# yangjames/Calico

Measured on AMD Instinct MI355X. Metric: LM iterations/sec on the 4-cam+IMU ~100k-observation problem, higher is better.
Workload: dtype f64

## Files before the change

calico_amd/csrc/bcr_kernels.hip:

```cpp
#include <hip/hip_runtime.h>

#include <algorithm>
#include <cassert>
#include <mutex>
#include <type_traits>

#include "kernels.hpp"
#include "problem_dev.hpp"
#include "solve_dev.hpp"
#include "block_elim.hpp"

namespace cal {

namespace {
constexpr int BP = kBcrBP;
constexpr int BB = BP * BP;
constexpr int DLD = 33;
constexpr int XLD = 2 * BP + kBcrFS + 1;
constexpr int CA = 0, CB = BP, CF = 2 * BP;
constexpr int kLevelThreads = 512;
constexpr int kLevelCodePrefetchBytes = 40 * 1024;
}

template <bool NEG, int NK>
// ... 63 lines not shown
struct Handoff { int* word; int seq; };
DEVI double load_sc1(const double* p) { return __hip_atomic_load(p, __ATOMIC_RELAXED, __HIP_MEMORY_SCOPE_AGENT); }
DEVI void store_sc1(double* p, double v) { __hip_atomic_store(p, v, __ATOMIC_RELAXED, __HIP_MEMORY_SCOPE_AGENT); }
template <bool HO> DEVI double load_y(const double* p) { return HO ? load_sc1(p) : *p; }
DEVI void handoff_publish(const Handoff& h) {
  asm volatile("s_waitcnt vmcnt(0)" ::: "memory");
  __syncthreads();
  if (threadIdx.x == 0) __hip_atomic_store(h.word, h.seq, __ATOMIC_RELAXED, __HIP_MEMORY_SCOPE_AGENT);
}
DEVI void fanin_arrive(int* word) {
  asm volatile("s_waitcnt vmcnt(0)" ::: "memory");
  __syncthreads();
  if (threadIdx.x == 0) __hip_atomic_fetch_add(word, 1, __ATOMIC_RELAXED, __HIP_MEMORY_SCOPE_AGENT);
}
DEVI void fanin_wait(const int* word, int n) {
  if (threadIdx.x == 0) {
    while (__hip_atomic_load(word, __ATOMIC_RELAXED, __HIP_MEMORY_SCOPE_AGENT) < n) __builtin_amdgcn_s_sleep(4);
  }
  __syncthreads();
}
DEVI void handoff_wait(const Handoff& h) {
  if (threadIdx.x == 0) {
    while (__hip_atomic_load(h.word, __ATOMIC_RELAXED, __HIP_MEMORY_SCOPE_AGENT) != h.seq) __builtin_amdgcn_s_sleep(4);
  }
  __syncthreads();
}

template <int NW, bool LATE>
DEVI void schur_tile(const SolveArgs& a, const BcrArgs& b, const FromR& fr, int tile, int slice, int ks, double* sacc ,
                     const int* fan_word, int n_prod, int late0, int late1) {
  const int mc = a.mc, m = a.m, m1 = a.m + 1, m1p = b.m1p, m1y = a.mc + 1;
  const int tid = threadIdx.x, lane = tid & 63, wave = tid >> 6;
  const size_t msq = size_t(m1) * m1;
  const int n = b.N * BP;
  int tr = 0, rem = tile;
  while (rem > tr) { rem -= tr + 1; ++tr; }
  const int tc = rem;
  const int lc16 = lane & 15, lk = lane >> 4;
  const int rows_per = ((n + ks - 1) / ks + 15) & ~15;
  const int r_begin = slice * rows_per, r_end = min(n, r_begin + rows_per);
  const int per_wave = (((r_end - r_begin + NW - 1) / NW + 3) / 4) * 4;
  const int w_begin = r_begin + wave * per_wave, w_end = min(r_end, w_begin + per_wave);
  const int ca = 16 * tr + lc16, cb = 16 * tc + lc16;
  const double* pa = b.Y + ca;
  const double* pb = b.Y + cb;
  const int f0 = LATE ? late0 : -1, f1 = LATE ? late1 : -1;
  double s0_pre = 0.0;
  if (tid < 256) {
    const int r = tr * 16 + (tid >> 4), c = tc * 16 + (tid & 15);
    if (r < m1y && c <= r && slice == 0) {
      if (r < mc) {
        s0_pre = a.R[a.off_C() + size_t(r) * mc + c];
        if (r == c) { const double d = fr.damping(s0_pre, a.n_s() + r); a.dadd[a.n_s() + r] = d; s0_pre += d; }
      } else if (c < mc) s0_pre = a.R[a.off_g() + a.n_s() + c];
    }
  }
  f64x4 acc = {0.0, 0.0, 0.0, 0.0};
  for (int kg = w_begin; kg < w_end; kg += 128) {
    double va[4][8], vb[4][8];
#pragma unroll
    for (int g = 0; g < 4; ++g) {
#pragma unroll
      for (int u = 0; u < 8; ++u) {
        const int row = kg + 32 * g + 4 * u + lk;
        const size_t ro = size_t(min(row, n - 1)) * m1p;
        va[g][u] = pa[ro]; vb[g][u] = pb[ro];
      }
    }
#pragma unroll
    for (int g = 0; g < 4; ++g) {
#pragma unroll
      for (int u = 0; u < 8; ++u) {
        const int row = kg + 32 * g + 4 * u + lk, sb = row >> 5;
        const bool use = row < w_end && sb != f0 && sb != f1;
        acc = __builtin_amdgcn_mfma_f64_16x16x4f64(use ? va[g][u] : 0.0, use ? vb[g][u] : 0.0, acc, 0, 0, 0);
      }
    }
  }
  if (LATE) {
    fanin_wait(fan_word, n_prod);
#pragma unroll
    for (int f = 0; f < 2; ++f) {
      const int sb = f == 0 ? f0 : f1;
      const int row = BP * max(sb, 0) + 4 * wave + lk;
      const bool use = sb >= 0 && wave < 8 && row >= r_begin && row < r_end;
      const size_t ro = size_t(min(row, n - 1)) * m1p;
      const double va = load_sc1(pa + ro), vb = load_sc1(pb + ro);
      acc = __builtin_amdgcn_mfma_f64_16x16x4f64(use ? va : 0.0, use ? vb : 0.0, acc, 0, 0, 0);
    }
  }
#pragma unroll
  for (int r = 0; r < 4; ++r) sacc[wave * 256 + (lk + 4 * r) * 16 + lc16] = acc[r];
  __syncthreads();
  if (tid < 256) {
    const int ti = tid >> 4, tj = tid & 15;
    const int r = tr * 16 + ti, c = tc * 16 + tj;
    double sum = 0.0;
#pragma unroll
    for (int w = 0; w < NW; ++w) sum += sacc[w * 256 + tid];
    if (r < m1y && c <= r) {
      const int fi = r < mc ? r : m, fc = c < mc ? c : m;
      a.Spart[size_t(slice) * msq + size_t(fi) * m1 + fc] = s0_pre - sum;
    }
  }
}
template <bool SC1>
DEVI void schur_root_rows(const SolveArgs& a, const BcrArgs& b, int ks, int w0, int nw, int NT) {
  if (b.root < 0) return;
  const int mc = a.mc, m = a.m, m1 = a.m + 1, m1p = b.m1p, m1y = a.mc + 1;
  const size_t msq = size_t(m1) * m1;
  const int tid = threadIdx.x;
  const int br = m - mc;
  const size_t fblk = size_t(BP) * m1p;
  const double* pD = b.pendD + size_t(b.root_par) * size_t(b.N) * 2 * BB;
  const double* pF = b.pendF + size_t(b.root_par) * size_t(b.N) * 2 * fblk;
  const int mask = b.root_pend;
  const int total = br * (m1y + br);
  auto ld = [](const double* p) { return SC1 ? load_sc1(p) : *p; };
  for (int e = w0 * NT + tid; e < total; e += nw * NT) {
    const int r = e / (m1y + br), j = e % (m1y + br);
    const bool in_f = j < m1y;
    const int r2 = j - m1y;
    if (!in_f && r2 > r) continue;
    const size_t o = in_f ? size_t(r) * m1p + j : size_t(r) * BP + r2;
    const double* base = in_f ? b.F + size_t(b.root) * fblk : b.D + size_t(b.root) * BB;
    const double* p0 = in_f ? pF + (size_t(b.root) * 2 + 0) * fblk : pD + (size_t(b.root) * 2 + 0) * BB;
    const double* p1 = in_f ? pF + (size_t(b.root) * 2 + 1) * fblk : pD + (size_t(b.root) * 2 + 1) * BB;
    const double v0 = ld(base + o), v1 = ld(p0 + o), v2 = ld(p1 + o);
    const double v = (v0 + ((mask & 1) ? v1 : 0.0)) + ((mask & 2) ? v2 : 0.0);
    int fi, fc;
    if (in_f) { if (j < mc) { fi = mc + r; fc = j; } else { fi = m; fc = mc + r; } }
    else { fi = mc + r; fc = mc + r2; }
    a.Spart[size_t(fi) * m1 + fc] = v;
    for (int k = 1; k < ks; ++k) a.Spart[size_t(k) * msq + size_t(fi) * m1 + fc] = 0.0;
  }
}

constexpr int kBcrTri = BP * (BP + 1) / 2;
template <int NL_, int NU_, int NF_>
struct BcrLoadMap {
  static constexpr int NL = NL_, NU = NU_, NF = NF_;
  static constexpr int NUD = (kBcrTri + NL_ - 1) / NL_;
  static_assert(NUD <= NU_ && NU_ <= 8 && NF_ <= 8, "BcrLoadMap: per-thread entry counts must fit the arrays and the flag bytes");
  int lt;
  int iD[NU_], iB[NU_];
  int rcD[NU_];
  bool okD[NU_], okB[NU_];
};
template <int NU, int NF>
struct BcrPre { double d[NU], bt[NU], at[NU], f[NF]; };
template <int NUD, int NU, int NF>
struct BcrRaw { double vraw[NUD], svv[NUD], q2v[NUD], vraw1[NUD], graw[NU], garaw[NU], graw1[NU], garaw1[NU], fraw[NF], fraw1[NF]; unsigned flags; };
constexpr int kRollTabWords = 48;
__device__ unsigned g_roll_tab[6][64][kRollTabWords];
static void fill_roll_table(unsigned (*tab)[64][kRollTabWords]) {
  constexpr int RB = 6 * kBcrCps;
  for (int k = 1; k <= 6; ++k) {
    auto pos = [&](int hi, int lo, bool& ok) {
      const int d = hi / 6 - lo / 6;
      ok = d < k;
      return unsigned(8 * (((lo / 6) * k + (ok ? d : 0)) * 36 + (lo % 6) * 6 + hi % 6));
    };
    for (int lane = 0; lane < 64; ++lane) {
      unsigned* t = tab[k - 1][lane];
      for (int i = 0; i < kRollTabWords; ++i) t[i] = 0;
      const int l16 = lane & 15, lk = lane >> 4;
      unsigned okS = 0, okB = 0, okA = 0;
      for (int r = 0; r < 4; ++r) {
        const int c = lk + 4 * r, hi = std::max(l16, c), lo = std::min(l16, c);
        bool ok;
        t[r] = pos(hi, lo, ok); if (ok) okS |= 1u << r;
        t[4 + r] = pos(16 + l16, c, ok); if (ok && 16 + l16 < RB) okS |= 1u << (4 + r);
        t[8 + r] = pos(16 + hi, 16 + lo, ok); if (ok && 16 + hi < RB) okS |= 1u << (8 + r);
      }
      for (int qt = 0; qt < 2; ++qt)
        for (int h = 0; h < 2; ++h)
          for (int r = 0; r < 4; ++r) {
            const int e = (qt * 2 + h) * 4 + r;
            bool ok;
            {
              const int c = 16 * h + lk + 4 * r, rn = 16 * qt + l16;
              t[12 + e] = pos(RB + rn, c, ok);
              if (ok && rn < RB && c < RB) okB |= 1u << e;
            }
            {
              const int rb = 16 * h + lk + 4 * r, cs = 16 * qt + l16;
              t[32 + e] = pos(RB + rb, cs, ok);
              if (ok && rb < RB && cs < RB) okA |= 1u << e;
            }
          }
      t[28] = okS | okB << 16;
      t[29] = okA;
    }
  }
}
void roll_table_row(int k, int lane, unsigned* out) {
  static unsigned tab[6][64][kRollTabWords];
  static std::once_flag once;
  std::call_once(once, [] { fill_roll_table(tab); });
  for (int i = 0; i < kRollTabWords; ++i) out[i] = tab[k - 1][lane][i];
}
hipError_t upload_roll_table() {
  static unsigned host_tab[6][64][kRollTabWords];
  static std::once_flag once;
  std::call_once(once, [] { fill_roll_table(host_tab); });
  return hipMemcpyToSymbol(HIP_SYMBOL(g_roll_tab), host_tab, sizeof(host_tab));
}

template <bool FROM_R, bool ELIM, bool ROLL = false>
__global__ __launch_bounds__(kLevelThreads) void bcr_level_kernel(SolveArgs a, BcrArgs b, int node0, int n_nodes, int nfs, int level,
                                                                   int keep0, int n_keep, LmOptionsDev o, int with_post,
                                                                   const double* __restrict__ x, const BlockDev* __restrict__ blocks,
                                                                   int n_blocks, IterLog* log, int log_cap, int jacobi_scaling,
                                                                   int n_schur_wg, int n_root_wg, int schur_ks, int* fan_word, int n_prod,
                                                                   BcrInlineNodes inl) {
  const long long t_kernel = CAL_DEV_TIMING(a.debug != 0) ? __builtin_readcyclecounter() : 0;
  LmState* st = a.st;
  const LmState* const stv = vector_ptr(const_cast<const LmState*>(st));
  const int terminated_v = stv->terminated;
  const double radius = stv->radius;
  const int r_cur_v = FROM_R ? stv->rcur : 0;
  uint4 tv[8], tva[4];
  if constexpr (ROLL) {
    const uint4* const tl = reinterpret_cast<const uint4*>(&g_roll_tab[min(max(a.k, 1), 6) - 1][threadIdx.x & 63][0]);
#pragma unroll
    for (int i = 0; i < 8; ++i) tv[i] = tl[i];
#pragma unroll
    for (int i = 0; i < 4; ++i) tva[i] = tl[8 + i];
  }
  int code_pf = 0;
  if constexpr (!ROLL) code_pf = prefetch_code(threadIdx.x, kLevelThreads, kLevelCodePrefetchBytes);
  const bool pub = !FROM_R && fan_word != nullptr;
  if (FROM_R && fan_word != nullptr && blockIdx.x == 0 && threadIdx.x == 0) *fan_word = 0;
  if (pub && int(blockIdx.x) >= int(gridDim.x) - n_schur_wg - n_root_wg) {
    if (uniform(terminated_v)) return;
    use_current_R(a);
    const FromR frs = {a, o, radius, 0};
    extern __shared__ double lds_s[];
    const int w = int(blockIdx.x) - (int(gridDim.x) - n_schur_wg - n_root_wg);
    if (w < n_schur_wg) {
      const int lb0 = inl.n > 0 ? inl.nd[0].blk0 : b.nodes[node0].blk0, lb1 = n_nodes > 1 ? (inl.n > 0 ? inl.nd[1].blk0 : b.nodes[node0 + 1].blk0) : -1;
      schur_tile<kLevelThreads / 64, true>(a, b, frs, w / schur_ks, w % schur_ks, schur_ks, lds_s, fan_word, n_prod, lb0, lb1);
      if (CAL_DEV_TIMING((a.debug == 4 || a.debug == 6) && threadIdx.x == 0 && w < 2)) printf("bcr_level %d: Schur tile rider %d lived %lld clocks\n", level, w, (long long)(__builtin_readcyclecounter() - t_kernel));
    } else {
      fanin_wait(fan_word, n_prod);
      const long long t_fan = CAL_DEV_TIMING(a.debug == 4 || a.debug == 6) ? __builtin_readcyclecounter() - t_kernel : 0;
      schur_root_rows<true>(a, b, schur_ks, w - n_schur_wg, n_root_wg, kLevelThreads);
      if (CAL_DEV_TIMING((a.debug == 4 || a.debug == 6) && threadIdx.x == 0 && w == n_schur_wg)) printf("bcr_level %d: root-row rider: fan-in complete at %lld clocks, lived %lld\n", level, t_fan, (long long)(__builtin_readcyclecounter() - t_kernel));
    }
    return;
  }
  auto put = [&](double* dst, double v) { if (pub) store_sc1(dst, v); else *dst = v; };
  if (FROM_R) {
    if (with_post && blockIdx.x == gridDim.x - 1) {
      if (uniform(terminated_v)) return;
      if (threadIdx.x == 0 && a.st->commit_pending) a.st->commit_pending = 0;
      post_eval_body(a, x, blocks, n_blocks, o, log, log_cap, with_post == 2 ? 1 : 0, jacobi_scaling);
      if (CAL_DEV_TIMING(a.debug == 4 && threadIdx.x == 0)) printf("bcr_level 0: the bookkeeping workgroup lived %lld clocks\n", (long long)(__builtin_readcyclecounter() - t_kernel));
      return;
    }
  }
  const double* const R_buf0 = a.R;
  const double* const R_buf1 = a.R + a.r_stride;
  const FromR fr = {a, o, radius, (FROM_R && with_post == 2) ? (jacobi_scaling ? 1 : 2) : 0};
  const int tid = threadIdx.x, lane = tid & 63, wave = __builtin_amdgcn_readfirstlane(tid >> 6);
  const int per = 1 + nfs;
  const int main_span = 8 * ((n_nodes + 7) / 8) * per;
  const int pcol = int(blockIdx.x) & 7, pslot = int(blockIdx.x) >> 3;
  const int node_l = (pslot / per) * 8 + pcol;
  const bool extra_wg = int(blockIdx.x) >= main_span;
  if (!extra_wg && node_l >= n_nodes) return;
  const int bid = extra_wg ? n_nodes * per + (int(blockIdx.x) - main_span) : node_l * per + pslot % per;
  const int grid_l = n_nodes * per + (int(gridDim.x) - n_schur_wg - n_root_wg - main_span);
  const int m1p = b.m1p, par = level & 1;
  const size_t NB = size_t(b.N);
  const size_t fblk = size_t(BP) * m1p;
  double* const pendD_w = b.pendD + size_t(par) * NB * 2 * BB;
  double* const pendF_w = b.pendF + size_t(par) * NB * 2 * fblk;
  const double* const pendD_r = b.pendD + size_t(par ^ 1) * NB * 2 * BB;
  const double* const pendF_r = b.pendF + size_t(par ^ 1) * NB * 2 * fblk;
  const double* const Gr = b.G + size_t(par) * NB * BB;
  double* const Gw = b.G + size_t(par ^ 1) * NB * BB;
  if (bid >= n_nodes * per) {
    if (uniform(terminated_v)) { if (pub) fanin_arrive(fan_word); return; }
    if (FROM_R) use_current_R(a);
    const size_t aw = size_t(bid - n_nodes * per), naw = size_t(grid_l - n_nodes * per - (FROM_R && with_post ? 1 : 0));
    const size_t per_blk = size_t(BB) + fblk;
    if (FROM_R) {
      const size_t total = size_t(n_keep) * per_blk, stride = naw * kLevelThreads;
      const int n_s = a.n_s();
      for (size_t e0 = aw * kLevelThreads + tid; e0 < total; e0 += 4 * stride) {
        size_t ridx[4], didx[4];
        int trd[4], flags[4];
#pragma unroll
        for (int u = 0; u < 4; ++u) {
          const size_t e = e0 + u * stride;
          const size_t ec = e < total ? e : total - 1;
          const int kb = int(ec / per_blk);
          const size_t rem = ec - size_t(kb) * per_blk;
          const int blk = b.keep[2 * (keep0 + kb)];
          int fl = e < total ? 1 : 0;
          size_t ri = 0;
          int tr_d = 0;
          if (rem < size_t(BB)) {
            const int r = int(rem) >> 5, c = int(rem) & 31;
            const int tr = fr.trow(blk, r), tc = fr.trow(blk, c);
            const int hi = max(tr, tc), lo = min(tr, tc);
            const int lo_c = max(lo, 0), ic = lo_c / 6, cc = lo_c % 6, ir = max(hi, 0) / 6, rr = max(hi, 0) % 6, d = ir - ic;
            const bool ok = lo >= 0 && d < a.k;
            ri = a.off_B() + (size_t(ic) * a.k + (ok ? d : 0)) * 36 + cc * 6 + rr;
            if (ok) fl |= 2;
            if (r == c) { fl |= 4; const int t = FromR::RB * blk + r; if (r < FromR::RB && t < n_s) fl |= 8; tr_d = tr >= 0 ? tr : -1 - (t < n_s ? t : 0); }
            didx[u] = size_t(blk) * BB + rem;
          } else {
            const size_t q = rem - BB;
            const int r = int(q / m1p), j = int(q % m1p);
            const int tr = fr.trow(blk, r), t = max(tr, 0), jc = min(j, a.mc);
            ri = j < a.mc ? a.off_E() + size_t(t) * a.mc + jc : a.off_g() + t;
            if (tr >= 0 && j <= a.mc) fl |= 2;
            fl |= 16;
            didx[u] = size_t(blk) * fblk + q;
          }
          ridx[u] = ri; trd[u] = tr_d; flags[u] = fl;
        }
        double rv[4], sc[4];
#pragma unroll
        for (int u = 0; u < 4; ++u) { rv[u] = a.R[ridx[u]]; sc[u] = a.scale[(flags[u] & 4) ? max(trd[u], 0) : 0]; }
#pragma unroll
        for (int u = 0; u < 4; ++u) {
          const int fl = flags[u];
          if (!(fl & 1)) continue;
          double v = (fl & 2) ? rv[u] : 0.0;
          if (fl & 4) {
            if (trd[u] >= 0) {
              const double sv = fr.first_scale == 0 ? sc[u] : fr.scale_of(v, 0);
              const double dd = fmin(fmax(v * sv * sv, o.min_lm_diagonal), o.max_lm_diagonal) / (radius * sv * sv);
              v += dd; a.dadd[trd[u]] = dd;
            } else {
              v = 1.0;
              if (fl & 8) a.dadd[-1 - trd[u]] = 0.0;
            }
          }
          if (fl & 16) b.F[didx[u]] = v; else b.D[didx[u]] = v;
        }
      }
      if (CAL_DEV_TIMING(a.debug == 4 && threadIdx.x == 0 && aw == 0)) printf("bcr_level 0: a separator-initialisation workgroup lived %lld clocks\n", (long long)(__builtin_readcyclecounter() - t_kernel));
      if (pub) fanin_arrive(fan_word);
      return;
    }
    for (size_t e = aw * kLevelThreads + tid; e < size_t(n_keep) * per_blk; e += naw * kLevelThreads) {
      const int kb = int(e / per_blk);
      const size_t rem = e % per_blk;
      const int blk = b.keep[2 * (keep0 + kb)], mask = b.keep[2 * (keep0 + kb) + 1];
      if (rem < size_t(BB)) {
        double v = b.D[size_t(blk) * BB + rem];
        if (mask & 1) v += pendD_r[(size_t(blk) * 2 + 0) * BB + rem];
        if (mask & 2) v += pendD_r[(size_t(blk) * 2 + 1) * BB + rem];
        put(b.D + size_t(blk) * BB + rem, v);
      } else {
        const size_t q = rem - BB;
        double v = b.F[size_t(blk) * fblk + q];
        if (mask & 1) v += pendF_r[(size_t(blk) * 2 + 0) * fblk + q];
        if (mask & 2) v += pendF_r[(size_t(blk) * 2 + 1) * fblk + q];
        put(b.F + size_t(blk) * fblk + q, v);
      }
    }
    if (pub) fanin_arrive(fan_word);
    return;
  }
  BcrNodeDev nd_;
  {
    const int c = bid / per;
    if (FROM_R && inl.q_regular > 0) {
      nd_.blk0 = c * (inl.q_regular + 1); nd_.q = min(inl.q_regular, b.N - nd_.blk0);
      nd_.left = c > 0 ? nd_.blk0 - 1 : -1; nd_.right = nd_.blk0 + nd_.q < b.N ? nd_.blk0 + nd_.q : -1; nd_.slot = node0 + c; nd_.pend = 0;
    } else if (!FROM_R && inl.n > 0) {
      nd_ = inl.nd[0];
      if (c == 1) nd_ = inl.nd[1];
      if (c == 2) nd_ = inl.nd[2];
      if (c == 3) nd_ = inl.nd[3];
    } else nd_ = b.nodes[node0 + c];
  }
// ... 130 lines not shown
#pragma unroll
      for (int u = 0; u < NF; ++u) rw.fraw[u] = second ? rw.fraw1[u] : rw.fraw[u];
    }
#pragma unroll
    for (int u = 0; u < NU; ++u) { pr.bt[u] = (fl >> (8 + u)) & 1 ? rw.graw[u] : 0.0; pr.at[u] = (fl >> (16 + u)) & 1 ? rw.garaw[u] : 0.0; }
#pragma unroll
    for (int u = 0; u < NUD; ++u) {
      const int r = m.rcD[u] >> 8, c = m.rcD[u] & 255;
      const bool vD = (fl >> u) & 1;
      double v = vD ? rw.vraw[u] : 0.0;
      {
        const bool dg = r == c;
        const int t = RB * blk + r;
        const bool real_row = r < RB && r < nreal;
        double d;
        const double inv_radius = 1.0 / radius;
        if (fr.first_scale == 0) d = fmin(fmax(v * rw.svv[u] * rw.svv[u], o.min_lm_diagonal), o.max_lm_diagonal) * (inv_radius * rw.q2v[u]);
        else d = fr.damping(v, (dg && real_row) ? t : 0);
        if (dg) {
          if (vD) { v += d; if (role == 0) a.dadd[t] = d; }
          else { v = 1.0; if (role == 0 && real_row) a.dadd[t] = 0.0; }
        }
      }
      pr.d[u] = v;
    }
#pragma unroll
    for (int u = 0; u < NF; ++u) pr.f[u] = (fl >> (24 + u)) & 1 ? rw.fraw[u] : 0.0;
  };
  auto fetch = [&](int i, auto& pr, auto both_tag, const auto& m) {
    typedef typename std::remove_reference<decltype(m)>::type M;
    constexpr int NL = M::NL, NU = M::NU, NF = M::NF;
    const int lt = m.lt;
    const int blk = blk0 + i, mask = pend_mask;
    const bool has_next = (i + 1 < q) || right >= 0;
    const bool has_a = (i == 0) && left >= 0;
    const size_t lc = size_t(left > 0 ? left : 0);
    if (FROM_R) {
      BcrRaw<M::NUD, NU, NF> rw;
      fetch_request(i, rw, both_tag, m);
      fetch_finish(i, rw, pr, both_tag, m);
      return;
    }
#pragma unroll
    for (int u = 0; u < NU; ++u) {
      const int e = min(max(lt, 0) + NL * u, BB - 1);
      const double v0 = b.D[size_t(blk) * BB + e];
      const double v1 = pendD_r[(size_t(blk) * 2 + 0) * BB + e];
      const double v2 = pendD_r[(size_t(blk) * 2 + 1) * BB + e];
      pr.d[u] = (v0 + ((mask & 1) ? v1 : 0.0)) + ((mask & 2) ? v2 : 0.0);
      const double g = Gr[size_t(blk) * BB + e];
      pr.bt[u] = has_next ? g : 0.0;
      double ga = 0.0;
      if (has_a) ga = Gr[lc * BB + e];
      pr.at[u] = ga;
    }
#pragma unroll
    for (int u = 0; u < NF; ++u) {
      const int e = min(max(lt, 0) + NL * u, BP * kBcrFS - 1);
      const int r = e >> 4, j = e & 15;
      const int col = role > 0 ? f0 + j : 0;
      const size_t o2 = size_t(r) * m1p + col;
      const double v0 = b.F[size_t(blk) * fblk + o2];
      const double v1 = pendF_r[(size_t(blk) * 2 + 0) * fblk + o2];
      const double v2 = pendF_r[(size_t(blk) * 2 + 1) * fblk + o2];
      pr.f[u] = role > 0 ? (v0 + ((mask & 1) ? v1 : 0.0)) + ((mask & 2) ? v2 : 0.0) : 0.0;
    }
  };
  auto commit = [&](int p, const auto& pr, const auto& m) {
    typedef typename std::remove_reference<decltype(m)>::type M;
    constexpr int NL = M::NL, NU = M::NU, NF = M::NF;
    const int lt = m.lt;
    double* Dp = Daug + p * 64 * DLD;
    double* Xp = Xb + p * BP * XLD;
    if (FROM_R) {
#pragma unroll
      for (int u = 0; u < M::NUD; ++u) {
        if (lt + NL * u < kBcrTri) {
          const int r = m.rcD[u] >> 8, c = m.rcD[u] & 255;
          Dp[r * DLD + c] = pr.d[u];
          if (r != c) Dp[c * DLD + r] = pr.d[u];
          if (!ELIM) { Dp[(BP + r) * DLD + c] = r == c ? 1.0 : 0.0; if (r != c) Dp[(BP + c) * DLD + r] = 0.0; }
        }
      }
#pragma unroll
      for (int u = 0; u < NU; ++u) {
        const int e = lt + NL * u;
        if (e < BB) {
          const int c = e >> 5, r = e & 31;
          Xp[c * XLD + CB + r] = pr.bt[u];
          Xp[r * XLD + CA + c] = pr.at[u];
        }
      }
    } else {
#pragma unroll
    for (int u = 0; u < NU; ++u) {
      const int e = lt + NL * u;
      if (e < BB) {
        const int r = e >> 5, c = e & 31;
        Dp[r * DLD + c] = pr.d[u];
        if (!ELIM) Dp[(BP + r) * DLD + c] = r == c ? 1.0 : 0.0;
        Xp[c * XLD + CB + r] = pr.bt[u];
        Xp[r * XLD + CA + c] = pr.at[u];
      }
    }
    }
#pragma unroll
    for (int u = 0; u < NF; ++u) {
      const int e = lt + NL * u;
      if (e < BP * kBcrFS) Xp[(e >> 4) * XLD + CF + (e & 15)] = pr.f[u];
    }
  };
  const bool dbg = CAL_DEV_TIMING(a.debug && a.debug < 4 && bid < 2 && lane == 0 && (wave == 0 || wave == 5));
  long long tph[8] = {0, 0, 0, 0, 0, 0, 0, 0}, tk = dbg ? __builtin_readcyclecounter() : 0;
  const long long t_setup = CAL_DEV_TIMING(a.debug >= 4) ? __builtin_readcyclecounter() - t_kernel : 0;
  long long t_first = 0, t_loop = 0, t_top[4] = {0, 0, 0, 0}, t_elim[4] = {0, 0, 0, 0}, t_bara[4] = {0, 0, 0, 0};
#define LTICK(i) if (dbg) { const long long t_ = __builtin_readcyclecounter(); tph[i] += t_ - tk; tk = t_; }
  double pmin = 1.0;
  f64x4 acc_a = {0.0, 0.0, 0.0, 0.0};
  if constexpr (ROLL) {
    constexpr int kImg = 28 * 64;
    double* const Zr = lds;
    double* const Mr = Zr + 2 * BP * XLD;
    double* const chb = Mr + 2 * BP * DLD;
    double* const img = chb + 3 * kElimBufDoubles;
    int* const ctr = reinterpret_cast<int*>(img + 2 * kImg);
    long long* const tstamp = reinterpret_cast<long long*>(ctr + 16);
    static_assert(2 * BP * XLD + 2 * BP * DLD + 3 * kElimBufDoubles + 2 * kImg + 8 + 64 + 16 <= 2 * 64 * DLD + 4 * BP * XLD + 80 + 128 + kLevelThreads + kElimBufDoubles,
                  "the rolling chief's LDS layout must fit the level kernels' allocation");
    enum { C_DONE_D0 = 0, C_DONE_D1 = 1, C_DONE_A = 2, C_DONE_F = 3, C_TAKEN_A = 4, C_TAKEN_F = 5, C_TAKEN_D0 = 6, C_TAKEN_D1 = 7, C_FILED = 8, C_STAGED = 12 };
    auto ctr_set = [&](int idx, int v) {
      asm volatile("" ::: "memory");
      if (lane == 0) __hip_atomic_store(ctr + idx, v, __ATOMIC_RELAXED, __HIP_MEMORY_SCOPE_WORKGROUP);
      asm volatile("" ::: "memory");
    };
    auto ctr_wait = [&](auto cond) {
      for (;;) {
        const int cv = __hip_atomic_load(ctr + (lane & 15), __ATOMIC_RELAXED, __HIP_MEMORY_SCOPE_WORKGROUP);
        if (cond([&](int i) { return __builtin_amdgcn_readlane(cv, i); })) break;
        __builtin_amdgcn_s_sleep(2);
      }
      asm volatile("" ::: "memory");
    };
    auto all4_ge = [&](auto& c, int base, int v) { return c(base) >= v && c(base + 1) >= v && c(base + 2) >= v && c(base + 3) >= v; };
    auto done_d = [&](auto& c, int j) { return c((j & 1) ? C_DONE_D0 : C_DONE_D1) >= j + 1; };
    const bool tdbg = CAL_DEV_TIMING(a.debug >= 4);
    auto stamp = [&](int k, int which) { if (tdbg && lane == 0 && k < 4) tstamp[(wave * 4 + k) * 2 + which] = __builtin_readcyclecounter() - t_kernel; };
    long long* const hs = tstamp + 64;
    auto hstamp = [&](int i) { if (tdbg && lane == 0 && wave < 2) hs[wave * 8 + i] = __builtin_readcyclecounter() - t_kernel; };
    hstamp(0);
    const f64x4 zero4 = {0.0, 0.0, 0.0, 0.0};
    const bool has_left = left >= 0;
    const int n_s = a.n_s(), kk = a.k;
    const bool tile_wave = wave < 2 || wave == 7;
    const unsigned tmask = tv[7].y;
    for (int e = tid; e < 3 * kElimBufDoubles; e += kLevelThreads) reinterpret_cast<unsigned long long*>(chb)[e] = kElimSentinel;
    if (tid < 16) ctr[tid] = 0;
    if (tdbg && tid < 64) tstamp[tid] = 0;
    hstamp(1);
    lds_barrier();
    hstamp(2);
    if (CAL_DEV_TIMING(a.debug == 5)) { asm volatile("s_waitcnt vmcnt(0)" ::: "memory"); hstamp(7); }
    const size_t alt = a.r_stride;
    const double* const bandR = R_buf0 + a.off_B();
    auto ldo = [](const double* base, unsigned byte_off) { return *reinterpret_cast<const double*>(reinterpret_cast<const char*>(base) + byte_off); };
    auto zops = [&](const double* Zb, int col0, double (&v)[8]) {
      const double* pp = Zb + lk * XLD + col0 + l16;
#pragma unroll
      for (int u = 0; u < 8; ++u) v[u] = pp[4 * u * XLD];
    };
    auto fill_half = [&](int jt) {
      ctr_wait([&](auto c) { return done_d(c, q - 1) && c(C_DONE_A) >= q; });
      const double* Zp = Zr + ((q - 1) & 1) * BP * XLD;
      double zb0[8], zb1[8], za[8];
      zops(Zp, CB, zb0); zops(Zp, CB + 16, zb1); zops(Zp, CA + 16 * jt, za);
      f64x4 g0 = zero4, g1 = zero4;
#pragma unroll
      for (int u = 0; u < 8; ++u) {
        g0 = __builtin_amdgcn_mfma_f64_16x16x4f64(-zb0[u], za[u], g0, 0, 0, 0);
        g1 = __builtin_amdgcn_mfma_f64_16x16x4f64(-zb1[u], za[u], g1, 0, 0, 0);
      }
      double* dst = Gw + size_t(left) * BB;
#pragma unroll
      for (int r = 0; r < 4; ++r) {
        dst[(lk + 4 * r) * BP + 16 * jt + l16] = g0[r];
        dst[(16 + lk + 4 * r) * BP + 16 * jt + l16] = g1[r];
      }
    };
    const bool want_fill = right >= 0 && has_left && role == 0;
    const bool all_act = b.all_active != 0;
    auto req_act = [&](int I) { return all_act ? 1 : int(a.cp_active[min(max(kBcrCps * I + (lane & 7), 0), a.n_cp - 1)]); };
    auto act_mask = [&](int flag) { return all_act ? 31u : (unsigned(__builtin_amdgcn_ballot_w64(flag != 0 && (lane & 7) < kBcrCps)) & 31u); };
    auto act = [](unsigned am, int row) { return ((am >> (row / 6)) & 1u) != 0; };
    if (tile_wave) {
      unsigned oS[12], oB[16];
#pragma unroll
      for (int i = 0; i < 3; ++i) { oS[4 * i] = tv[i].x; oS[4 * i + 1] = tv[i].y; oS[4 * i + 2] = tv[i].z; oS[4 * i + 3] = tv[i].w; }
#pragma unroll
      for (int i = 0; i < 4; ++i) { oB[4 * i] = tv[3 + i].x; oB[4 * i + 1] = tv[3 + i].y; oB[4 * i + 2] = tv[3 + i].z; oB[4 * i + 3] = tv[3 + i].w; }
      const unsigned okS = tv[7].x & 0xffffu, okB = tv[7].x >> 16;
      const bool diag_lane = l16 >= lk && ((l16 - lk) & 3) == 0;
      struct Inputs { double sp[12], sc[4], bt[16]; int fa, fn; };
      auto req_scale = [&](int I, double (&sc)[4]) {
        const int nreal = n_s - RB * I;
        const unsigned t0 = (diag_lane && l16 < nreal) ? RB * I + l16 : 0, t1 = (diag_lane && 16 + l16 < RB && 16 + l16 < nreal) ? RB * I + 16 + l16 : 0;
        sc[0] = ldo(a.scale, 8u * t0); sc[1] = ldo(a.scale + a.NT(), 8u * t0); sc[2] = ldo(a.scale, 8u * t1); sc[3] = ldo(a.scale + a.NT(), 8u * t1);
      };
      auto req_spine = [&](int I, double (&sp)[12], const double* base) {
        const double* p = base + size_t(I) * strideB;
#pragma unroll
        for (int e = 0; e < 12; ++e) sp[e] = ldo(p, oS[e]);
      };
      auto req_b = [&](int J, double (&bt)[16], const double* base) {
        const double* p = base + size_t(J) * strideB;
#pragma unroll
        for (int e = 0; e < 16; ++e) bt[e] = ldo(p, oB[e]);
      };
      const double inv_radius = 1.0 / radius;
      auto take_spine_t = [&](auto act_tag, int I, const double (&sp)[12], const double (&sc)[4], unsigned am, f64x4& t00, f64x4& t01, f64x4& t11) {
        constexpr bool ACT = decltype(act_tag)::value;
        auto act = [](unsigned m_, int row) { return !ACT || ((m_ >> (row / 6)) & 1u) != 0; };
        const int nreal = n_s - RB * I;
        double e00[4], e01[4], e11[4];
        const bool a0 = act(am, l16), a1 = act(am, 16 + l16);
#pragma unroll
        for (int r = 0; r < 4; ++r) {
          const int c = lk + 4 * r, hi = max(l16, c);
          const bool v00 = ((okS >> r) & 1) && hi < nreal && a0 && act(am, c), v01 = ((okS >> (4 + r)) & 1) && 16 + l16 < nreal && a1 && act(am, c),
                     v11 = ((okS >> (8 + r)) & 1) && 16 + hi < nreal && a1 && act(am, 16 + c);
          e00[r] = v00 ? sp[r] : 0.0; e01[r] = v01 ? sp[4 + r] : 0.0; e11[r] = v11 ? sp[8 + r] : 0.0;
        }
        const int dr = (l16 - lk) >> 2;
        double dg[2];
        dg[0] = dr == 1 ? e00[1] : (dr == 2 ? e00[2] : (dr == 3 ? e00[3] : e00[0]));
        dg[1] = dr == 1 ? e11[1] : (dr == 2 ? e11[2] : (dr == 3 ? e11[3] : e11[0]));
#pragma unroll
        for (int h = 0; h < 2; ++h) {
          const int row = 16 * h + l16, t = RB * I + row;
          const bool in_traj = row < RB && row < nreal, real_row = in_traj && (h == 0 ? a0 : a1);
          double d;
          if (fr.first_scale == 0) d = fmin(fmax(dg[h] * sc[2 * h] * sc[2 * h], o.min_lm_diagonal), o.max_lm_diagonal) * (inv_radius * sc[2 * h + 1]);
          else d = fr.damping(dg[h], real_row ? t : 0);
          if (diag_lane && in_traj && role == 0) a.dadd[t] = real_row ? d : 0.0;
          dg[h] = real_row ? dg[h] + d : 1.0;
        }
#pragma unroll
        for (int r = 0; r < 4; ++r) {
          const bool is_d = diag_lane && dr == r;
          t00[r] = -(is_d ? dg[0] : e00[r]); t01[r] = -e01[r]; t11[r] = -(is_d ? dg[1] : e11[r]);
        }
      };
      auto take_spine = [&](int I, const double (&sp)[12], const double (&sc)[4], unsigned am, f64x4& t00, f64x4& t01, f64x4& t11) {
        if (all_act) take_spine_t(std::false_type(), I, sp, sc, am, t00, t01, t11); else take_spine_t(std::true_type(), I, sp, sc, am, t00, t01, t11);
      };
      auto take_b_t = [&](auto act_tag, int k, const double (&bt)[16], unsigned am_this, unsigned am_next, f64x4 (&x0)[2], f64x4 (&x1)[2]) {
        constexpr bool ACT = decltype(act_tag)::value;
        auto act = [](unsigned m_, int row) { return !ACT || ((m_ >> (row / 6)) & 1u) != 0; };
        const bool has_next = (k + 1 < q) || right >= 0;
        const int nreal_n = n_s - RB * (blk0 + k + 1);
#pragma unroll
        for (int qt = 0; qt < 2; ++qt) {
          const bool row_ok = has_next && 16 * qt + l16 < nreal_n && act(am_next, 16 * qt + l16);
#pragma unroll
          for (int r = 0; r < 4; ++r) {
            x0[qt][r] = -((((okB >> ((qt * 2 + 0) * 4 + r)) & 1) && row_ok && act(am_this, lk + 4 * r)) ? bt[(qt * 2 + 0) * 4 + r] : 0.0);
            x1[qt][r] = -((((okB >> ((qt * 2 + 1) * 4 + r)) & 1) && row_ok && act(am_this, 16 + lk + 4 * r)) ? bt[(qt * 2 + 1) * 4 + r] : 0.0);
          }
        }
      };
      auto take_b = [&](int k, const double (&bt)[16], unsigned am_this, unsigned am_next, f64x4 (&x0)[2], f64x4 (&x1)[2]) {
        if (all_act) take_b_t(std::false_type(), k, bt, am_this, am_next, x0, x1); else take_b_t(std::true_type(), k, bt, am_this, am_next, x0, x1);
      };
      if (wave < 2) {
        const int par = wave;
        f64x4 t00 = zero4, t01 = zero4, t11 = zero4;
        f64x4 x0[2], x1[2], n00 = zero4, n01 = zero4, n11 = zero4;
        {
          Inputs in, alt_in;
          if (par == 0) {
            req_spine(blk0, in.sp, bandR); req_spine(blk0, alt_in.sp, bandR + alt); req_scale(blk0, in.sc);
            in.fn = req_act(blk0); in.fa = in.fn;
          } else {
            req_b(blk0, in.bt, bandR); req_b(blk0, alt_in.bt, bandR + alt);
            if (q > 1) { req_spine(blk0 + 1, in.sp, bandR); req_spine(blk0 + 1, alt_in.sp, bandR + alt); req_scale(blk0 + 1, in.sc); }
            in.fa = req_act(blk0); in.fn = req_act(blk0 + 1);
          }
          hstamp(3);
          if (uniform(terminated_v)) return;
          hstamp(4);
          const bool second = uniform(r_cur_v) != 0;
#pragma unroll
          for (int e = 0; e < 12; ++e) in.sp[e] = second ? alt_in.sp[e] : in.sp[e];
          if (tdbg) { asm volatile("s_waitcnt vmcnt(0)" ::: "memory"); hstamp(5); }
          const unsigned ma = act_mask(in.fa), mn = act_mask(in.fn);
          if (par == 0) take_spine(blk0, in.sp, in.sc, mn, t00, t01, t11);
          else {
#pragma unroll
            for (int e = 0; e < 16; ++e) in.bt[e] = second ? alt_in.bt[e] : in.bt[e];
            take_b(0, in.bt, ma, mn, x0, x1);
            if (q > 1) take_spine(blk0 + 1, in.sp, in.sc, mn, n00, n01, n11);
          }
          hstamp(6);
        }
        for (int k = 0; k < q; ++k) {
          const ElimChannel chk = elim_channel(chb + (k % 3) * kElimBufDoubles);
          if ((k & 1) == par) {
            stamp(k, 0);
            elim_chief_reg<0>(t00, t01, t11, nullptr, 0, chk, lane);
            stamp(k, 1);
          } else {
            if (k > 0) {
              ctr_wait([&](auto c) { return c(C_STAGED) >= k + 1 && (k < 2 || (all4_ge(c, C_FILED, k - 1) && c(C_TAKEN_A) >= k && (role == 0 || c(C_TAKEN_F) >= k))); });
              const double* im = img + (k & 1) * kImg + lane;
#pragma unroll
              for (int r = 0; r < 4; ++r) {
                n00[r] = im[(0 + r) * 64]; n01[r] = im[(4 + r) * 64]; n11[r] = im[(8 + r) * 64];
                x0[0][r] = im[(12 + r) * 64]; x1[0][r] = im[(16 + r) * 64]; x0[1][r] = im[(20 + r) * 64]; x1[1][r] = im[(24 + r) * 64];
              }
              ctr_set(par == 0 ? C_TAKEN_D0 : C_TAKEN_D1, k + 1);
            }
            stamp(k, 0);
            double* const Zk = Zr + (k & 1) * BP * XLD;
            elim_follow_d(x0, x1, Zk + CB, Zk + CB + 16, 1, XLD, chk, lane, n00, n01, n11);
            ctr_set(par == 0 ? C_DONE_D0 : C_DONE_D1, k + 1);
            stamp(k, 1);
            if (k + 1 < q) { t00 = n00; t01 = n01; t11 = n11; }
            else if (right >= 0 && role == 0) {
              double* dst = pendD_w + (size_t(right) * 2 + 0) * BB;
#pragma unroll
              for (int r = 0; r < 4; ++r) {
                const int c = lk + 4 * r;
                dst[c * BP + l16] = -n00[r];
                dst[(16 + l16) * BP + c] = -n01[r];
                dst[(16 + c) * BP + 16 + l16] = -n11[r];
              }
            }
          }
        }
        if (want_fill && par == ((q - 1) & 1)) fill_half(1);
      } else {
        if (uniform(terminated_v)) return;
        a.R = uniform(r_cur_v) ? R_buf1 : R_buf0;
        const double* const bandC = a.R + a.off_B();
        const int lt2 = tid - 256;
        for (int k = 0; k < q; ++k) {
          const int j = k + 1;
          if (j < q) {
            stamp(k, 0);
            Inputs in;
            req_b(blk0 + j, in.bt, bandC);
            if (j + 1 < q) { req_spine(blk0 + j + 1, in.sp, bandC); req_scale(blk0 + j + 1, in.sc); }
            in.fa = req_act(blk0 + j); in.fn = req_act(blk0 + j + 1);
            f64x4 x0[2], x1[2], n00 = zero4, n01 = zero4, n11 = zero4;
            const unsigned ma = act_mask(in.fa), mn = act_mask(in.fn);
            take_b(j, in.bt, ma, mn, x0, x1);
            if (j + 1 < q) take_spine(blk0 + j + 1, in.sp, in.sc, mn, n00, n01, n11);
            if (j >= 3) ctr_wait([&](auto c) { return c((j & 1) ? C_TAKEN_D0 : C_TAKEN_D1) >= j - 1; });
            double* im = img + (j & 1) * kImg + lane;
#pragma unroll
            for (int r = 0; r < 4; ++r) {
              im[(0 + r) * 64] = n00[r]; im[(4 + r) * 64] = n01[r]; im[(8 + r) * 64] = n11[r];
              im[(12 + r) * 64] = x0[0][r]; im[(16 + r) * 64] = x1[0][r]; im[(20 + r) * 64] = x0[1][r]; im[(24 + r) * 64] = x1[1][r];
            }
            ctr_set(C_STAGED, j + 1);
            stamp(k, 1);
          }
          ctr_wait([&](auto c) { return done_d(c, k) && c(C_DONE_A) >= k + 1 && c(C_DONE_F) >= k + 1; });
          const int blk = blk0 + k;
          const double* const Zk = Zr + (k & 1) * BP * XLD;
          if (role == 0) {
            const double* const Mk = Mr + (k & 1) * BP * DLD;
#pragma unroll
            for (int u = 0; u < 4; ++u) {
              const int e = lt2 + 256 * u, r = e >> 5, c = e & 31;
              b.M[size_t(blk) * BB + e] = Mk[r * DLD + c];
              b.ZA[size_t(blk) * BB + e] = Zk[r * XLD + CA + c];
              b.ZB[size_t(blk) * BB + e] = Zk[r * XLD + CB + c];
            }
          } else {
#pragma unroll
            for (int u = 0; u < 2; ++u) { const int e = lt2 + 256 * u; b.Y[size_t(blk) * fblk + size_t(e >> 4) * m1p + f0 + (e & 15)] = Zk[(e >> 4) * XLD + CF + (e & 15)]; }
          }
          {
            unsigned long long* cp = reinterpret_cast<unsigned long long*>(chb + (k % 3) * kElimBufDoubles);
            for (int e = lt2; e < kElimBufDoubles; e += 256) cp[e] = kElimSentinel;
          }
          ctr_set(C_FILED + 3, k + 1);
        }
      }
    } else if (wave == 2) {
      f64x4 pre0[2] = {zero4, zero4}, pre1[2] = {zero4, zero4};
      {
        double av[16], av1[16];
        unsigned oA[16];
#pragma unroll
        for (int i = 0; i < 4; ++i) { oA[4 * i] = tva[i].x; oA[4 * i + 1] = tva[i].y; oA[4 * i + 2] = tva[i].z; oA[4 * i + 3] = tva[i].w; }
        const double* p = bandR + size_t(max(blk0 - 1, 0)) * strideB;
#pragma unroll
        for (int e = 0; e < 16; ++e) {
          av[e] = 0.0; av1[e] = 0.0;
          if (has_left) { av[e] = ldo(p, oA[e]); av1[e] = ldo(p + alt, oA[e]); }
        }
        const int f_this = req_act(blk0), f_left = req_act(blk0 - 1);
        if (uniform(terminated_v)) return;
        const bool second = uniform(r_cur_v) != 0;
        const int nreal = n_s - RB * blk0;
        const unsigned m_this = act_mask(f_this), m_left = act_mask(f_left);
#pragma unroll
        for (int qt = 0; qt < 2; ++qt) {
#pragma unroll
          for (int r = 0; r < 4; ++r) {
            const int e0 = (qt * 2 + 0) * 4 + r, e1 = (qt * 2 + 1) * 4 + r;
            const bool col_ok = has_left && act(m_left, 16 * qt + l16);
            const bool v0 = ((tmask >> e0) & 1) && col_ok && lk + 4 * r < nreal && act(m_this, lk + 4 * r),
                       v1 = ((tmask >> e1) & 1) && col_ok && 16 + lk + 4 * r < nreal && act(m_this, 16 + lk + 4 * r);
            pre0[qt][r] = -(v0 ? (second ? av1[e0] : av[e0]) : 0.0);
            pre1[qt][r] = -(v1 ? (second ? av1[e1] : av[e1]) : 0.0);
          }
        }
      }
      auto fill_pre = [&](const double* Zp) {
        double zb0[8], zb1[8], za[8];
        zops(Zp, CB, zb0); zops(Zp, CB + 16, zb1);
#pragma unroll
        for (int jt = 0; jt < 2; ++jt) {
          zops(Zp, CA + 16 * jt, za);
#pragma unroll
          for (int r = 0; r < 4; ++r) { pre0[jt][r] = -0.0; pre1[jt][r] = -0.0; }
#pragma unroll
          for (int u = 0; u < 8; ++u) {
            pre0[jt] = __builtin_amdgcn_mfma_f64_16x16x4f64(zb0[u], za[u], pre0[jt], 0, 0, 0);
            pre1[jt] = __builtin_amdgcn_mfma_f64_16x16x4f64(zb1[u], za[u], pre1[jt], 0, 0, 0);
          }
        }
      };
      for (int k = 0; k < q; ++k) {
        const ElimChannel chk = elim_channel(chb + (k % 3) * kElimBufDoubles);
        double* const Zk = Zr + (k & 1) * BP * XLD;
        if (k > 0) {
          ctr_wait([&](auto c) { return done_d(c, k - 1); });
          stamp(k, 0);
          if (has_left) fill_pre(Zr + ((k - 1) & 1) * BP * XLD);
        } else stamp(k, 0);
        ctr_set(C_TAKEN_A, k + 1);
        if (k >= 2) ctr_wait([&](auto c) { return all4_ge(c, C_FILED, k - 1); });
        const ElimTile t[2] = {{Zk, 0, 0, Zk + CA, 1, XLD, 0, nullptr}, {Zk, 0, 0, Zk + CA + 16, 1, XLD, 0, nullptr}};
        elim_follow<2>(t, chk, lane, true, pre0, pre1);
        ctr_set(C_DONE_A, k + 1);
        stamp(k, 1);
      }
      if (want_fill) fill_half(0);
    } else if (wave == 3) {
      if (role == 0) {
        if (uniform(terminated_v)) return;
        for (int k = 0; k < q; ++k) {
          const ElimChannel chk = elim_channel(chb + (k % 3) * kElimBufDoubles);
          double* const Mk = Mr + (k & 1) * BP * DLD;
          if (k >= 2) ctr_wait([&](auto c) { return all4_ge(c, C_FILED, k - 1); });
          stamp(k, 0);
          const ElimTile t[2] = {{Mk, 0, 0, Mk, DLD, 1, 1, nullptr}, {Mk, 0, 0, Mk + 16 * DLD, DLD, 1, 2, nullptr}};
          elim_follow<2>(t, chk, lane);
          ctr_set(C_DONE_F, k + 1);
          stamp(k, 1);
        }
      } else {
        f64x4 pre0[1], pre1[1];
        const int col = f0 + l16;
        auto req_f = [&](int k, double (&fv)[8], const double* Rb) {
          const int nreal = n_s - RB * (blk0 + k);
#pragma unroll
          for (int e = 0; e < 8; ++e) {
            const int r = 16 * (e >> 2) + lk + 4 * (e & 3), t = RB * (blk0 + k) + r;
            const bool vF = r < RB && r < nreal && col <= a.mc;
            fv[e] = Rb[vF ? (col < a.mc ? a.off_E() + size_t(t) * a.mc + col : a.off_g() + t) : a.off_g()];
          }
        };
        unsigned m_f = 31u;
        auto f_valid = [&](int k, int e) {
          const int r = 16 * (e >> 2) + lk + 4 * (e & 3);
          return r < RB && r < n_s - RB * (blk0 + k) && col <= a.mc && act(m_f, r);
        };
        double fv[8];
        int f_flag = req_act(blk0);
        {
          double fv1[8];
          req_f(0, fv, R_buf0); req_f(0, fv1, R_buf1);
          if (uniform(terminated_v)) return;
          const bool second = uniform(r_cur_v) != 0;
          a.R = second ? R_buf1 : R_buf0;
#pragma unroll
          for (int e = 0; e < 8; ++e) fv[e] = second ? fv1[e] : fv[e];
        }
        for (int k = 0; k < q; ++k) {
          const ElimChannel chk = elim_channel(chb + (k % 3) * kElimBufDoubles);
          double* const Zk = Zr + (k & 1) * BP * XLD;
          if (k > 0) ctr_wait([&](auto c) { return done_d(c, k - 1); });
          stamp(k, 0);
          m_f = act_mask(f_flag);
#pragma unroll
          for (int r = 0; r < 4; ++r) { pre0[0][r] = -(f_valid(k, r) ? fv[r] : 0.0); pre1[0][r] = -(f_valid(k, 4 + r) ? fv[4 + r] : 0.0); }
          if (k + 1 < q) { req_f(k + 1, fv, a.R); f_flag = req_act(blk0 + k + 1); }
          if (k > 0) {
            const double* Zp = Zr + ((k - 1) & 1) * BP * XLD;
            double zb0[8], zb1[8], zf[8];
            zops(Zp, CB, zb0); zops(Zp, CB + 16, zb1); zops(Zp, CF, zf);
#pragma unroll
            for (int u = 0; u < 8; ++u) {
              pre0[0] = __builtin_amdgcn_mfma_f64_16x16x4f64(zb0[u], zf[u], pre0[0], 0, 0, 0);
              pre1[0] = __builtin_amdgcn_mfma_f64_16x16x4f64(zb1[u], zf[u], pre1[0], 0, 0, 0);
            }
          }
          ctr_set(C_TAKEN_F, k + 1);
          if (k >= 2) ctr_wait([&](auto c) { return all4_ge(c, C_FILED, k - 1); });
          const ElimTile t[1] = {{Zk, 0, 0, Zk + CF, 1, XLD, 0, nullptr}};
          elim_follow<1>(t, chk, lane, true, pre0, pre1);
          ctr_set(C_DONE_F, k + 1);
          stamp(k, 1);
        }
        if (right >= 0) {
          ctr_wait([&](auto c) { return done_d(c, q - 1); });
          const double* Zp = Zr + ((q - 1) & 1) * BP * XLD;
          double zb0[8], zb1[8], zf[8];
          zops(Zp, CB, zb0); zops(Zp, CB + 16, zb1); zops(Zp, CF, zf);
          f64x4 s0 = zero4, s1 = zero4;
#pragma unroll
          for (int u = 0; u < 8; ++u) {
            s0 = __builtin_amdgcn_mfma_f64_16x16x4f64(-zb0[u], zf[u], s0, 0, 0, 0);
            s1 = __builtin_amdgcn_mfma_f64_16x16x4f64(-zb1[u], zf[u], s1, 0, 0, 0);
          }
          double* dst = pendF_w + (size_t(right) * 2 + 0) * fblk + f0 + l16;
#pragma unroll
          for (int r = 0; r < 4; ++r) { put(dst + size_t(lk + 4 * r) * m1p, s0[r]); put(dst + size_t(16 + lk + 4 * r) * m1p, s1[r]); }
        }
      }
    } else {
      if (uniform(terminated_v)) return;
      const int w4 = wave - 4, lt2 = tid - 256;
      const bool acc_owner = wave == 5 || wave == 6, acc_owner2 = role == 0 && wave == 5;
      const int acc_p = role == 0 ? CA + (wave == 6 ? 16 : 0) : CA + 16 * (wave - 5);
      const int acc_q = role == 0 ? CA + (wave == 6 ? 16 : 0) : CF;
      f64x4 acc2 = zero4;
      for (int k = 0; k < q; ++k) {
        ctr_wait([&](auto c) { return done_d(c, k) && c(C_DONE_A) >= k + 1 && c(C_DONE_F) >= k + 1; });
        stamp(k, 0);
        const int blk = blk0 + k;
        const double* const Zk = Zr + (k & 1) * BP * XLD;
        if (role == 0) {
          const double* const Mk = Mr + (k & 1) * BP * DLD;
#pragma unroll
          for (int u = 0; u < 4; ++u) {
            const int e = lt2 + 256 * u, r = e >> 5, c = e & 31;
            b.M[size_t(blk) * BB + e] = Mk[r * DLD + c];
            b.ZA[size_t(blk) * BB + e] = Zk[r * XLD + CA + c];
            b.ZB[size_t(blk) * BB + e] = Zk[r * XLD + CB + c];
          }
        } else {
#pragma unroll
          for (int u = 0; u < 2; ++u) { const int e = lt2 + 256 * u; put(b.Y + size_t(blk) * fblk + size_t(e >> 4) * m1p + f0 + (e & 15), Zk[(e >> 4) * XLD + CF + (e & 15)]); }
        }
        if (has_left && acc_owner) acc_a = atb_tile<true>(Zk, XLD, acc_p, Zk, XLD, acc_q, 0, BP, acc_a, lane);
        if (has_left && acc_owner2) acc2 = atb_tile<true>(Zk, XLD, CA + 16, Zk, XLD, CA, 0, BP, acc2, lane);
        {
          unsigned long long* cp = reinterpret_cast<unsigned long long*>(chb + (k % 3) * kElimBufDoubles);
          for (int e = lt2; e < kElimBufDoubles; e += 256) cp[e] = kElimSentinel;
        }
        ctr_set(C_FILED + w4, k + 1);
        stamp(k, 1);
      }
      if (has_left) {
        if (role == 0) {
// ... 1721 lines not shown
```

Measured before the change: 10470.

## Lane-interleave roll table, load only active R buffer, overlap head barrier with loads

Transposes the roll lookup table so that each wave's per-lane uint4 loads are coalesced, and wave 2 loads only the four words it needs. Band loads now select the current R buffer up front by reading rcur, rather than loading both buffers and picking one per element, which halves global traffic and register use. The LDS head barrier is moved after the loads are issued so their latency overlaps the barrier, and only waves 4-6 clear the channel buffers. The cost is a dependence on rcur before the loads and more complex barrier placement across waves.

```diff
diff --git a/calico_amd/csrc/bcr_kernels.hip b/calico_amd/csrc/bcr_kernels.hip
--- a/calico_amd/csrc/bcr_kernels.hip
+++ b/calico_amd/csrc/bcr_kernels.hip
@@ -239,7 +239,7 @@
 template <int NUD, int NU, int NF>
 struct BcrRaw { double vraw[NUD], svv[NUD], q2v[NUD], vraw1[NUD], graw[NU], garaw[NU], graw1[NU], garaw1[NU], fraw[NF], fraw1[NF]; unsigned flags; };
 constexpr int kRollTabWords = 48;
-__device__ unsigned g_roll_tab[6][64][kRollTabWords];
+__device__ uint4 g_roll_tab[6][kRollTabWords / 4][64];
 static void fill_roll_table(unsigned (*tab)[64][kRollTabWords]) {
   constexpr int RB = 6 * kBcrCps;
   for (int k = 1; k <= 6; ++k) {
@@ -289,9 +289,18 @@
 }
 hipError_t upload_roll_table() {
   static unsigned host_tab[6][64][kRollTabWords];
+  static uint4 dev_tab[6][kRollTabWords / 4][64];
   static std::once_flag once;
-  std::call_once(once, [] { fill_roll_table(host_tab); });
-  return hipMemcpyToSymbol(HIP_SYMBOL(g_roll_tab), host_tab, sizeof(host_tab));
+  std::call_once(once, [] {
+    fill_roll_table(host_tab);
+    for (int k = 0; k < 6; ++k)
+      for (int lane = 0; lane < 64; ++lane)
+        for (int w = 0; w < kRollTabWords / 4; ++w) {
+          const unsigned* t = host_tab[k][lane] + 4 * w;
+          dev_tab[k][w][lane] = make_uint4(t[0], t[1], t[2], t[3]);
+        }
+  });
+  return hipMemcpyToSymbol(HIP_SYMBOL(g_roll_tab), dev_tab, sizeof(dev_tab));
 }
 
 template <bool FROM_R, bool ELIM, bool ROLL = false>
@@ -307,14 +316,13 @@
   const int terminated_v = stv->terminated;
   const double radius = stv->radius;
   const int r_cur_v = FROM_R ? stv->rcur : 0;
-  uint4 tv[8], tva[4];
+  uint4 tw[8];
   if constexpr (ROLL) {
-    const uint4* const tl = reinterpret_cast<const uint4*>(&g_roll_tab[min(max(a.k, 1), 6) - 1][threadIdx.x & 63][0]);
-#pragma unroll
-    for (int i = 0; i < 8; ++i) tv[i] = tl[i];
-#pragma unroll
-    for (int i = 0; i < 4; ++i) tva[i] = tl[8 + i];
-  }
+    const uint4* const tl = &g_roll_tab[min(max(a.k, 1), 6) - 1][(threadIdx.x >> 6) == 2 ? 4 : 0][threadIdx.x & 63];
+#pragma unroll
+    for (int i = 0; i < 8; ++i) tw[i] = tl[64 * i];
+  }
+  const uint4 (&tv)[8] = tw;
   int code_pf = 0;
   if constexpr (!ROLL) code_pf = prefetch_code(threadIdx.x, kLevelThreads, kLevelCodePrefetchBytes);
   const bool pub = !FROM_R && fan_word != nullptr;
@@ -751,13 +759,16 @@
     const bool has_left = left >= 0;
     const int n_s = a.n_s(), kk = a.k;
     const bool tile_wave = wave < 2 || wave == 7;
-    const unsigned tmask = tv[7].y;
-    for (int e = tid; e < 3 * kElimBufDoubles; e += kLevelThreads) reinterpret_cast<unsigned long long*>(chb)[e] = kElimSentinel;
+    static_assert((3 * kElimBufDoubles) % 192 == 0, "waves 4..6 clear the three channels in whole passes");
+    if (wave >= 4 && wave < 7) {
+      unsigned long long* const cp = reinterpret_cast<unsigned long long*>(chb) + (tid - 256);
+#pragma unroll
+      for (int u = 0; u < 3 * kElimBufDoubles / 192; ++u) cp[192 * u] = kElimSentinel;
+    }
     if (tid < 16) ctr[tid] = 0;
     if (tdbg && tid < 64) tstamp[tid] = 0;
-    hstamp(1);
-    lds_barrier();
-    hstamp(2);
+    auto head_barrier = [&] { hstamp(1); lds_barrier(); hstamp(2); };
+    if (wave > 2) head_barrier();
     if (CAL_DEV_TIMING(a.debug == 5)) { asm volatile("s_waitcnt vmcnt(0)" ::: "memory"); hstamp(7); }
     const size_t alt = a.r_stride;
     const double* const bandR = R_buf0 + a.off_B();
@@ -874,27 +885,24 @@
         f64x4 t00 = zero4, t01 = zero4, t11 = zero4;
         f64x4 x0[2], x1[2], n00 = zero4, n01 = zero4, n11 = zero4;
         {
-          Inputs in, alt_in;
+          Inputs in;
+          const double* const bandH = uniform(r_cur_v) != 0 ? bandR + alt : bandR;
+          hstamp(4);
           if (par == 0) {
-            req_spine(blk0, in.sp, bandR); req_spine(blk0, alt_in.sp, bandR + alt); req_scale(blk0, in.sc);
+            req_spine(blk0, in.sp, bandH); req_scale(blk0, in.sc);
             in.fn = req_act(blk0); in.fa = in.fn;
           } else {
-            req_b(blk0, in.bt, bandR); req_b(blk0, alt_in.bt, bandR + alt);
-            if (q > 1) { req_spine(blk0 + 1, in.sp, bandR); req_spine(blk0 + 1, alt_in.sp, bandR + alt); req_scale(blk0 + 1, in.sc); }
+            req_b(blk0, in.bt, bandH);
+            if (q > 1) { req_spine(blk0 + 1, in.sp, bandH); req_scale(blk0 + 1, in.sc); }
             in.fa = req_act(blk0); in.fn = req_act(blk0 + 1);
           }
           hstamp(3);
+          head_barrier();
           if (uniform(terminated_v)) return;
-          hstamp(4);
-          const bool second = uniform(r_cur_v) != 0;
-#pragma unroll
-          for (int e = 0; e < 12; ++e) in.sp[e] = second ? alt_in.sp[e] : in.sp[e];
           if (tdbg) { asm volatile("s_waitcnt vmcnt(0)" ::: "memory"); hstamp(5); }
           const unsigned ma = act_mask(in.fa), mn = act_mask(in.fn);
           if (par == 0) take_spine(blk0, in.sp, in.sc, mn, t00, t01, t11);
           else {
-#pragma unroll
-            for (int e = 0; e < 16; ++e) in.bt[e] = second ? alt_in.bt[e] : in.bt[e];
             take_b(0, in.bt, ma, mn, x0, x1);
             if (q > 1) take_spine(blk0 + 1, in.sp, in.sc, mn, n00, n01, n11);
           }
@@ -989,19 +997,20 @@
     } else if (wave == 2) {
       f64x4 pre0[2] = {zero4, zero4}, pre1[2] = {zero4, zero4};
       {
-        double av[16], av1[16];
+        double av[16];
         unsigned oA[16];
 #pragma unroll
-        for (int i = 0; i < 4; ++i) { oA[4 * i] = tva[i].x; oA[4 * i + 1] = tva[i].y; oA[4 * i + 2] = tva[i].z; oA[4 * i + 3] = tva[i].w; }
-        const double* p = bandR + size_t(max(blk0 - 1, 0)) * strideB;
+        for (int i = 0; i < 4; ++i) { oA[4 * i] = tw[4 + i].x; oA[4 * i + 1] = tw[4 + i].y; oA[4 * i + 2] = tw[4 + i].z; oA[4 * i + 3] = tw[4 + i].w; }
+        const unsigned tmask = tw[3].y;
+        const double* p = (uniform(r_cur_v) != 0 ? bandR + alt : bandR) + size_t(max(blk0 - 1, 0)) * strideB;
 #pragma unroll
         for (int e = 0; e < 16; ++e) {
-          av[e] = 0.0; av1[e] = 0.0;
-          if (has_left) { av[e] = ldo(p, oA[e]); av1[e] = ldo(p + alt, oA[e]); }
+          av[e] = 0.0;
+          if (has_left) av[e] = ldo(p, oA[e]);
         }
         const int f_this = req_act(blk0), f_left = req_act(blk0 - 1);
+        head_barrier();
         if (uniform(terminated_v)) return;
-        const bool second = uniform(r_cur_v) != 0;
         const int nreal = n_s - RB * blk0;
         const unsigned m_this = act_mask(f_this), m_left = act_mask(f_left);
 #pragma unroll
@@ -1012,8 +1021,8 @@
             const bool col_ok = has_left && act(m_left, 16 * qt + l16);
             const bool v0 = ((tmask >> e0) & 1) && col_ok && lk + 4 * r < nreal && act(m_this, lk + 4 * r),
                        v1 = ((tmask >> e1) & 1) && col_ok && 16 + lk + 4 * r < nreal && act(m_this, 16 + lk + 4 * r);
-            pre0[qt][r] = -(v0 ? (second ? av1[e0] : av[e0]) : 0.0);
-            pre1[qt][r] = -(v1 ? (second ? av1[e1] : av[e1]) : 0.0);
+            pre0[qt][r] = -(v0 ? av[e0] : 0.0);
+            pre1[qt][r] = -(v1 ? av[e1] : 0.0);
           }
         }
       }
```

Measured after the change: 10580 (median of 6 runs). About the same (+1.0%).
